# LeapLabTHU/LAUDNet

Measured on AMD Instinct MI355X. Metric: images/sec, LAUD-ResNet101 @224 bs256 (dynamic-inference hot path), higher is better.
Workload: dtype bf16x3 (fp32 tensors; each fp32 product = 3 bf16 MFMA products of hi/lo splits, fp32 accumulate)

## Files before the change

laudnet_amd/csrc/ldn_dense.hip:

```cpp
#include "ldn_common.h"
#include "ldn_dense_plan.h"
#include <type_traits>

namespace ldn {

struct DenseArgs {
    const float* a; int lda;
    const int32_t* a_rows; const int32_t* m_count; int m_cap;
    const unsigned char* ws;
    int cin, cout;
    const float* scale; const float* shift; int relu;
    const int32_t* relu_if_neg; const int32_t* out_rows;
    const float* residual; int ldr; float* out; int ldo;
    int taps;
    int shift_classes; const int32_t* pix_map;
    int Hi, Wi, Ho, Wo, stride;
    const float* post_sub;
    const float* chmask; int rows_per_img;
    int mtn, ntn;
    const float* ln_stats; const float* ln_c1;
    float* pool; int pool_gy, pool_gx, pool_Sx;
    const float* a_gate; int gate_rows;
};

__device__ __attribute__((aligned(16))) float g_dense_zero[2048] = {0.f};
#ifdef LDN_TRACE
__device__ unsigned long long* g_dense_trace = nullptr;
#define DT(x) x = __builtin_amdgcn_s_memtime();
#else
#define DT(x)
#endif

#ifndef LDN_DENSE_ABLATE
#define LDN_DENSE_ABLATE 0
#endif
__device__ __forceinline__ void dma16_abl(const void* gsrc, unsigned lds_base) {
#if LDN_DENSE_ABLATE & 1
    return;
#endif
#if LDN_DENSE_ABLATE & 2
    gsrc = g_dense_zero;
#endif
    dma16(gsrc, lds_base);
}

constexpr int D_ROWS_MAX = 256;
constexpr int D_ROW_RELU = 1 << 30;

template <int NSUB, bool T9, bool FULL, bool OF, bool FEAT = true>
__device__ __forceinline__ void dense_epilogue(const DenseArgs& p, f32x16 (&acc)[NSUB], const int* s_arow, const int* s_orow, const int* s_cls,
                                               float* scr, int wave, int lane, int n0, int nsub) {
    const int l31 = lane & 31, h = lane >> 5;
    const int trw = lane >> 3, tc = lane & 7;
    int orw[4];
#pragma unroll
    for (int it = 0; it < 4; ++it) orw[it] = s_orow[wave * 32 + trw + 8 * it];
    const bool gelu = FEAT && p.relu == 3;
    long poff = -1;
    const int pb3 = (lane >> 3) & 1, pb4 = (lane >> 4) & 1;
    if constexpr (!T9 && FULL) {
        if (p.pool) {
            const int it_sel = p.pool_gy * p.pool_gx == 16 ? (lane >= 32 ? 2 : 0) : pb3 + 2 * pb4;
            const int o = it_sel == 0 ? orw[0] : it_sel == 1 ? orw[1] : it_sel == 2 ? orw[2] : orw[3];
            if (o >= 0 && (p.pool_gy * p.pool_gx == 4 || (lane & 0x18) == 0)) {
                const int f = o & (D_ROW_RELU - 1), hw = p.Ho * p.Wo;
                const int b = f / hw, pix = f - b * hw, y = pix / p.Wo, x = pix - y * p.Wo;
                poff = ((long)b * (p.Ho / p.pool_gy) * p.pool_Sx + (y / p.pool_gy) * p.pool_Sx + x / p.pool_gx) * p.cout;
            }
        }
    }
    auto load_res = [&](int j, f32x4 (&res)[4], f32x4& sc, f32x4& sh, f32x4& ps) {
        const int cb = n0 + 32 * j + tc * 4;
        const bool cok = FULL || cb < p.cout;
#pragma unroll
        for (int it = 0; it < 4; ++it) {
            const float* src = (p.residual && orw[it] >= 0 && cok) ? p.residual + (size_t)(orw[it] & (D_ROW_RELU - 1)) * p.ldr + cb : g_dense_zero;
            res[it] = *reinterpret_cast<const f32x4*>(src);
        }
        sh = cok ? *reinterpret_cast<const f32x4*>(p.shift + cb) : f32x4{0.f, 0.f, 0.f, 0.f};
        sc = (p.scale && cok) ? *reinterpret_cast<const f32x4*>(p.scale + cb) : f32x4{1.f, 1.f, 1.f, 1.f};
        ps = (FEAT && p.post_sub && cok) ? *reinterpret_cast<const f32x4*>(p.post_sub + cb) : f32x4{0.f, 0.f, 0.f, 0.f};
    };
#pragma unroll
    for (int j = 0; j < NSUB; ++j) {
        if (j >= nsub) continue;
        f32x4 res[4], sc, sh, ps;
        load_res(j, res, sc, sh, ps);
        f32x4 cm[4];
        const bool cok = FULL || n0 + 32 * j + tc * 4 < p.cout;
        float2 lst[4];
        f32x4 lc1 = {0.f, 0.f, 0.f, 0.f};
        if (FEAT && p.ln_stats) {
#pragma unroll
            for (int it = 0; it < 4; ++it) {
                const int ar = s_arow[wave * 32 + trw + 8 * it];
                lst[it] = ar >= 0 ? *reinterpret_cast<const float2*>(p.ln_stats + 2 * (size_t)ar) : float2{0.f, 1.f};
            }
            if (cok) lc1 = *reinterpret_cast<const f32x4*>(p.ln_c1 + n0 + 32 * j + tc * 4);
        }
#pragma unroll
        for (int it = 0; it < 4; ++it) {
            const float* src = (FEAT && p.chmask && orw[it] >= 0 && cok) ? p.chmask + (size_t)((orw[it] & (D_ROW_RELU - 1)) / p.rows_per_img) * p.cout + n0 + 32 * j + tc * 4
                                                          : nullptr;
            cm[it] = src ? *reinterpret_cast<const f32x4*>(src) : f32x4{1.f, 1.f, 1.f, 1.f};
        }
#pragma unroll
        for (int q4 = 0; q4 < 4; ++q4) {
            const f32x4 v = {acc[j][4 * q4], acc[j][4 * q4 + 1], acc[j][4 * q4 + 2], acc[j][4 * q4 + 3]};
            *reinterpret_cast<f32x4*>(scr + l31 * 32 + (((2 * q4 + h) ^ (l31 & 7)) << 2)) = v;
        }
        asm volatile("s_waitcnt lgkmcnt(0)" ::: "memory");
        __builtin_amdgcn_wave_barrier();
        asm volatile("" : "+v"(res[0]), "+v"(res[1]), "+v"(res[2]), "+v"(res[3]), "+v"(sc), "+v"(sh), "+v"(ps));
        asm volatile("" : "+v"(cm[0]), "+v"(cm[1]), "+v"(cm[2]), "+v"(cm[3]));
        f32x4 xs4[4];
#pragma unroll
        for (int it = 0; it < 4; ++it) {
            const int row = trw + 8 * it;
            f32x4 x = *reinterpret_cast<const f32x4*>(scr + row * 32 + ((tc ^ (row & 7)) << 2));
            const f32x4 shr = (T9 && p.shift_classes > 1 && cok) ? *reinterpret_cast<const f32x4*>(p.shift + s_cls[wave * 32 + row] + n0 + 32 * j + tc * 4) : sh;
            if (FEAT && p.ln_stats) x = (x - lc1 * lst[it].x) * lst[it].y;
            x = x * sc + shr + res[it];
            if (orw[it] & D_ROW_RELU) {
#pragma unroll
                for (int e = 0; e < 4; ++e) x[e] = fmaxf(x[e], 0.f);
            }
            if (gelu) {
#pragma unroll
                for (int e = 0; e < 4; ++e) x[e] = 0.5f * x[e] * (1.f + erff(x[e] * 0.70710678118654752f));
            }
            x = (x - ps) * cm[it];
            if constexpr (OF) {
                const bool odd = tc & 1;
                const u32x4 o = presplit_store_quad(x, odd);
                if (orw[it] >= 0 && cok)
                    store16(reinterpret_cast<unsigned char*>(p.out) + ((size_t)(orw[it] & (D_ROW_RELU - 1)) * p.ldo + n0 + 32 * j + (tc & ~1) * 4) * 4 + (odd ? 16 : 0), o);
            } else {
                if (orw[it] >= 0 && cok)
                    store16(p.out + (size_t)(orw[it] & (D_ROW_RELU - 1)) * p.ldo + n0 + 32 * j + tc * 4, x);
            }
            xs4[it] = x;
        }
        if constexpr (!T9 && FULL) {
            if (p.pool) {
                auto swap32_sum = [](float a, float b) {
                    asm volatile("s_nop 1\n\tv_permlane32_swap_b32 %0, %1" : "+v"(a), "+v"(b));
                    return a + b;
                };
                auto swap16_sum = [](float a, float b) {
                    asm volatile("s_nop 1\n\tv_permlane16_swap_b32 %0, %1" : "+v"(a), "+v"(b));
                    return a + b;
                };
                auto ror8 = [](float a) { return __builtin_bit_cast(float, __builtin_amdgcn_update_dpp(0, __builtin_bit_cast(int, a), 0x128, 0xf, 0xf, false)); };
                f32x4 m;
                if (p.pool_gy * p.pool_gx == 16) {
                    const f32x4 sa = xs4[0] + xs4[1], sb = xs4[2] + xs4[3];
#pragma unroll
                    for (int e = 0; e < 4; ++e) {
                        float v = swap32_sum(sa[e], sb[e]);
                        v = swap16_sum(v, v);
                        m[e] = v + ror8(v);
                    }
                    m *= 0.0625f;
                } else {
                    const f32x4 k0 = pb3 ? xs4[1] : xs4[0], g0 = pb3 ? xs4[0] : xs4[1];
                    const f32x4 k2 = pb3 ? xs4[3] : xs4[2], g2 = pb3 ? xs4[2] : xs4[3];
#pragma unroll
                    for (int e = 0; e < 4; ++e) {
                        const float k01 = k0[e] + ror8(g0[e]), k23 = k2[e] + ror8(g2[e]);
                        m[e] = swap16_sum(k01, k23);
                    }
                    m *= 0.25f;
                }
                if (poff >= 0) *reinterpret_cast<f32x4*>(p.pool + poff + n0 + 32 * j + tc * 4) = m;
            }
        }
        asm volatile("s_waitcnt lgkmcnt(0)" ::: "memory");
        __builtin_amdgcn_wave_barrier();
    }
}

template <int NSUB, bool T9, bool FULL, bool F32 = false, int R = 256, bool PS = false, bool OF = false>
__global__ __launch_bounds__(2 * R, 2) void k_dense(const DenseArgs p) {
    constexpr int NT = NSUB * 32;
    constexpr int D = (NSUB >= 6 || R == 128) ? 2 : 3;
    constexpr int D_ROWS = R, NTHR = 2 * R, WR = R / 4;
    constexpr int SLOT = (D_ROWS + NT) * 128;
    constexpr int NWI = (NT + WR - 1) / WR;
    extern __shared__ __attribute__((aligned(16))) unsigned char smem[];
    int* const s_arow = reinterpret_cast<int*>(smem);
    int* const s_orow = s_arow + D_ROWS;
    int* const s_cls = s_orow + D_ROWS;
    int* const s_atap = s_cls + D_ROWS;
    unsigned char* const s_ring = smem + (T9 ? 12 : 2) * D_ROWS * 4;

    const int tid = threadIdx.x, lane = tid & 63;
    const int wave = __builtin_amdgcn_readfirstlane(tid >> 6);
    const int l31 = lane & 31, h = lane >> 5;
    const int xcd = blockIdx.x & 7, slot_i = blockIdx.x >> 3;
    const int nt = slot_i % p.ntn, mt = (slot_i / p.ntn) * 8 + xcd;
    if (mt >= p.mtn) return;
    const int M = p.m_count ? min(p.m_count[0], p.m_cap) : p.m_cap;
    const int m0 = mt * D_ROWS;
    if (m0 >= M) return;
    const int rows = min(D_ROWS, M - m0);
    const int n0 = nt * NT;
    const int nsub = FULL ? NSUB : min(NSUB, ceil_div(p.cout - n0, 32));

    if (tid < D_ROWS) {
        int ar = -1, orw = -1;
        if (tid < rows) {
            ar = (p.a_rows && !T9) ? p.a_rows[m0 + tid] : m0 + tid;
            orw = p.out_rows ? p.out_rows[m0 + tid] : m0 + tid;
            if (p.relu == 1 || (p.relu == 2 && p.relu_if_neg[m0 + tid] < 0)) orw |= D_ROW_RELU;
        }
        int cls = 0;
        if (T9 && tid < rows && p.shift_classes > 1) {
            const int q = p.pix_map[m0 + tid] % (p.Ho * p.Wo);
            const int oy = q / p.Wo, ox = q - oy * p.Wo;
            const int top = oy * p.stride - 1 < 0, bot = oy * p.stride + 1 >= p.Hi;
            const int lef = ox * p.stride - 1 < 0, rig = ox * p.stride + 1 >= p.Wi;
            cls = ((top | (bot << 1)) * 4 + (lef | (rig << 1))) * p.cout;
        }
        LDN_DCHECK(tid >= rows || (ar >= -1 && (orw & (D_ROW_RELU - 1)) >= 0), 501);
        s_arow[tid] = ar;
        s_orow[tid] = orw;
        if (T9) s_cls[tid] = cls;
    }
    if (T9) {
        constexpr int NE = (D_ROWS * 9 + NTHR - 1) / NTHR;
        int tv[NE];
#pragma unroll
        for (int u = 0; u < NE; ++u) {
            const int i = tid + NTHR * u, r = i / 9;
            tv[u] = (i < D_ROWS * 9 && r < rows) ? p.a_rows[(size_t)(m0 + r) * 9 + (i - r * 9)] : -1;
        }
#pragma unroll
        for (int u = 0; u < NE; ++u)
            if (tid + NTHR * u < D_ROWS * 9) s_atap[tid + NTHR * u] = tv[u];
    }
    __syncthreads();

    const bool active = wave * 32 < rows;
    const int cpt = ceil_div(p.cin, 32);
    const int wrow = (T9 ? 9 : 1) * (p.cin / 8);
    const int nchunks = (T9 ? 9 : 1) * cpt;
    const unsigned lds_ring = lds_off(s_ring);
    const int nwi = (NT % WR == 0 || (NWI - 1) * WR + wave * 8 < NT) ? NWI : NWI - 1;
    const int per_chunk = (active ? 4 : 0) + nwi;
    long asrc[4];
#pragma unroll
    for (int i = 0; i < 4; ++i) {
        const int ar = s_arow[wave * 32 + i * 8 + (lane >> 3)];
        asrc[i] = ar >= 0 ? (long)ar * p.lda : -1;
    }
    auto dma_chunk = [&](int c) {
        const unsigned slot = lds_ring + (c % D) * SLOT;
        const int tap = T9 ? c / cpt : 0, ck = c - tap * cpt;
        if (active) {
#pragma unroll
            for (int i = 0; i < 4; ++i) {
                const int r = wave * 32 + i * 8 + (lane >> 3);
                const int ls = (lane & 7) ^ ((r >> 1) & 7);
                long off = asrc[i];
                if (T9) {
                    const int ar = s_atap[r * 9 + tap];
// ... 92 lines not shown
        wait_vm_rt<16, 0>(per_chunk * (D - 2));
        DT(d1)
        lds_barrier();
        DT(d2)
        if (!(FULL && active)) { if (c + D - 1 < nchunks) dma_chunk(c + D - 1); else dma_dummy(c + D - 1); }
        DT(d3)
        if (!active) continue;
        const unsigned char* ws = s_ring + (c % D) * SLOT + D_ROWS * 128;
        if (!PRE) load_b(c);
#define LDN_DENSE_STEP(ACC_, AH_, AL_, BH_, BL_) \
        if constexpr (F32) { \
            const f32x4 a0_ = __builtin_bit_cast(f32x4, AH_), a1_ = __builtin_bit_cast(f32x4, AL_); \
            const f32x4 b0_ = __builtin_bit_cast(f32x4, BH_), b1_ = __builtin_bit_cast(f32x4, BL_); \
            _Pragma("unroll") for (int i_ = 0; i_ < 4; ++i_) ACC_ = __builtin_amdgcn_mfma_f32_32x32x2f32(a0_[i_], b0_[i_], ACC_, 0, 0, 0); \
            _Pragma("unroll") for (int i_ = 0; i_ < 4; ++i_) ACC_ = __builtin_amdgcn_mfma_f32_32x32x2f32(a1_[i_], b1_[i_], ACC_, 0, 0, 0); \
        } else { \
            ACC_ = __builtin_amdgcn_mfma_f32_32x32x16_bf16(AL_, BH_, ACC_, 0, 0, 0); \
            ACC_ = __builtin_amdgcn_mfma_f32_32x32x16_bf16(AH_, BL_, ACC_, 0, 0, 0); \
            ACC_ = __builtin_amdgcn_mfma_f32_32x32x16_bf16(AH_, BH_, ACC_, 0, 0, 0); \
        }
#ifdef LDN_TRACE
        asm volatile("" : "+v"(bh[0]), "+v"(bl[0]), "+v"(bh[1]), "+v"(bl[1]));
        DT(d4)
#endif
        auto frag = [&](int step, bf16x8& ah, bf16x8& al) {
            const int half = step / NSUB, j = step - half * NSUB;
            const unsigned sl = 4u * half + 2u * h;
#if LDN_DENSE_ABLATE & 8
            if (step > 1) return;
#endif
            ah = *reinterpret_cast<const bf16x8*>(ws + (32 * j + l31) * 128 + ((sl ^ wsw) << 4));
            al = *reinterpret_cast<const bf16x8*>(ws + (32 * j + l31) * 128 + (((sl + 1) ^ wsw) << 4));
        };
        if constexpr (FULL) {
            bf16x8 ah[2], al[2];
            frag(0, ah[0], al[0]);
            __builtin_amdgcn_sched_barrier(0);
#pragma unroll
            for (int st = 0; st < 2 * NSUB; ++st) {
                if (st + 1 < 2 * NSUB) frag(st + 1, ah[(st + 1) & 1], al[(st + 1) & 1]);
                __builtin_amdgcn_sched_barrier(0);
                const int half = st / NSUB, j = st - half * NSUB;
#if LDN_DENSE_ABLATE & 4
                asm volatile("" : "+v"(acc[j]) : "v"(al[st & 1]), "v"(ah[st & 1]), "v"(bh[half]), "v"(bl[half]));
#else
                LDN_DENSE_STEP(acc[j], ah[st & 1], al[st & 1], bh[half], bl[half])
#endif
                __builtin_amdgcn_sched_barrier(0);
                if (st < 4 + nwi) {
                    dma_one(c + D - 1, st);
                    __builtin_amdgcn_sched_barrier(0);
                }
            }
#pragma unroll
            for (int k = 2 * NSUB; k < 4 + NWI; ++k)
                if (k < 4 + nwi) dma_one(c + D - 1, k);
            if (PRE && c + 1 < nchunks) {
                wait_vm_rt<16, 0>(own_landed <= 16 ? own_landed : 0);
                load_b(c + 1);
            }
        } else {
#pragma unroll
            for (int half = 0; half < 2; ++half) {
#pragma unroll
                for (int j = 0; j < NSUB; ++j) {
                    if (j < nsub) {
                        bf16x8 ah, al;
                        frag(half * NSUB + j, ah, al);
                        LDN_DENSE_STEP(acc[j], ah, al, bh[half], bl[half])
                    }
                }
            }
        }
#ifdef LDN_TRACE
        asm volatile("" : "+v"(acc[0]));
        DT(d5)
        a_wait += d1 - d0; a_bar += d2 - d1; a_issue += d3 - d2; a_prep += d4 - d3; a_mfma += d5 - d4;
#endif
    }
#undef LDN_DENSE_STEP
#ifdef LDN_TRACE
    DT(d_loop)
#endif
    wait_vm<0>();
    lds_barrier();
    if (!active) return;

    dense_epilogue<NSUB, T9, FULL, OF>(p, acc, s_arow, s_orow, s_cls, reinterpret_cast<float*>(s_ring + wave * 4096), wave, lane, n0, nsub);
#if defined(LDN_TRACE)
    if (g_dense_trace && lane == 0) {
        unsigned long long dend;
        DT(dend)
        unsigned long long* r = g_dense_trace + ((size_t)blockIdx.x * 8 + wave) * 8;
        r[0] = a_wait; r[1] = a_bar; r[2] = a_issue; r[3] = a_prep; r[4] = a_mfma; r[5] = d_loop - d_start; r[6] = dend - d_loop; r[7] = nchunks;
    }
#endif
}

template <int NSUB, bool T9, bool PS, bool OF, bool FEAT = false, bool RAG = false, bool AG = false>
__global__ __launch_bounds__(512, 2) void k_dense2(const DenseArgs p) {
    static_assert(!RAG || (!T9 && !PS && !OF), "the ragged form is the plain 1x1");
    static_assert(!AG || (!T9 && !PS), "the gated form reads fp32 rows of a 1x1");
    constexpr int NT = NSUB * 32;
    constexpr int KS = NSUB <= 4 ? 64 : 32;
    constexpr int SPS = KS / 32;
    constexpr int WROWB = KS * 4;
    constexpr int UPR = WROWB / 16;
    constexpr int RPI = 1024 / WROWB;
    constexpr int NWI = (NT + 8 * RPI - 1) / (8 * RPI);
    constexpr int WSLOT = NWI * 8 * 1024;
    constexpr int RSLOT = 32 * 128;
    constexpr int D_ROWS = 256, NST = 2 * NSUB;
    extern __shared__ __attribute__((aligned(16))) unsigned char smem[];
    int* const s_arow = reinterpret_cast<int*>(smem);
    int* const s_orow = s_arow + D_ROWS;
    int* const s_cls = s_orow + D_ROWS;
    int* const s_atap = s_cls + D_ROWS;
    unsigned char* const s_w = smem + (T9 ? 12 : 2) * D_ROWS * 4;
    unsigned char* const s_r = s_w + 2 * WSLOT;
    float* const s_gate = reinterpret_cast<float*>(s_r + 8 * 2 * RSLOT);

    const int tid = threadIdx.x, lane = tid & 63;
    const int wave = __builtin_amdgcn_readfirstlane(tid >> 6);
    const int l31 = lane & 31, h = lane >> 5;
    const int xcd = blockIdx.x & 7, slot_i = blockIdx.x >> 3;
    const int nt = slot_i % p.ntn, mt = (slot_i / p.ntn) * 8 + xcd;
    if (mt >= p.mtn) return;
    const int M = p.m_count ? min(p.m_count[0], p.m_cap) : p.m_cap;
    const int m0 = mt * D_ROWS;
    if (m0 >= M) return;
    const int rows = min(D_ROWS, M - m0);
    const int n0 = nt * NT;

    if (tid < D_ROWS) {
        int ar = -1, orw = -1;
        if (tid < rows) {
            ar = (p.a_rows && !T9) ? p.a_rows[m0 + tid] : m0 + tid;
            orw = p.out_rows ? p.out_rows[m0 + tid] : m0 + tid;
            if (p.relu == 1 || (p.relu == 2 && p.relu_if_neg[m0 + tid] < 0)) orw |= D_ROW_RELU;
        }
        int cls = 0;
        if (T9 && tid < rows && p.shift_classes > 1) {
            const int q = p.pix_map[m0 + tid] % (p.Ho * p.Wo);
            const int oy = q / p.Wo, ox = q - oy * p.Wo;
            const int top = oy * p.stride - 1 < 0, bot = oy * p.stride + 1 >= p.Hi;
            const int lef = ox * p.stride - 1 < 0, rig = ox * p.stride + 1 >= p.Wi;
            cls = ((top | (bot << 1)) * 4 + (lef | (rig << 1))) * p.cout;
        }
        LDN_DCHECK(tid >= rows || (ar >= -1 && (orw & (D_ROW_RELU - 1)) >= 0), 501);
        s_arow[tid] = ar;
        s_orow[tid] = orw;
        if (T9) s_cls[tid] = cls;
    }
    if (T9) {
        constexpr int NE = (D_ROWS * 9 + 511) / 512;
        int tv[NE];
#pragma unroll
        for (int u = 0; u < NE; ++u) {
            const int i = tid + 512 * u, r = i / 9;
            tv[u] = (i < D_ROWS * 9 && r < rows) ? p.a_rows[(size_t)(m0 + r) * 9 + (i - r * 9)] : -1;
        }
#pragma unroll
        for (int u = 0; u < NE; ++u)
            if (tid + 512 * u < D_ROWS * 9) s_atap[tid + 512 * u] = tv[u];
    }
    int goff = 0;
    if constexpr (AG) {
        const int gld = round_up(p.cin, 32), q4 = gld >> 2;
        const int slot0 = m0 / p.gate_rows, nsl = (m0 + rows - 1) / p.gate_rows - slot0 + 1;
        for (int i = tid; i < nsl * q4; i += 512) {
            const int sl = i / q4, k = (i - sl * q4) * 4;
            reinterpret_cast<f32x4*>(s_gate)[i] = k < p.cin ? *reinterpret_cast<const f32x4*>(p.a_gate + (size_t)(slot0 + sl) * p.cin + k) : f32x4{0.f, 0.f, 0.f, 0.f};
        }
        goff = ((m0 + min(wave * 32 + (lane & 31), rows - 1)) / p.gate_rows - slot0) * gld + 8 * (lane >> 5);
    }
    __syncthreads();

    const bool active = wave * 32 < rows;
    const int cpt = RAG ? ceil_div(p.cin, 32) : p.cin >> 5;
    const int nsubc = (T9 ? 9 : 1) * cpt, nstep = RAG ? ceil_div(nsubc, SPS) : nsubc / SPS;
    const int nsub_t = RAG ? min(NSUB, ceil_div(p.cout - n0, 32)) : NSUB;
    const long wrow = (long)(T9 ? 9 : 1) * p.cin * 4;
    const unsigned lds_w = lds_off(s_w), lds_r = lds_off(s_r) + (unsigned)wave * 2u * RSLOT;
// ... 108 lines not shown

    load_tap(0);
#pragma unroll
    for (int k = 0; k < NWI; ++k) dma_w(0, k);
#pragma unroll
    for (int k = 0; k < 4; ++k) dma_r(0, k);
    next_r();
#pragma unroll
    for (int k = 0; k < 4; ++k) dma_r(1, k);
    next_r();
    wait_vm<4>();
    read_b(0, bh[0], bl[0]);
    split_b(0, bh[0], bl[0]);
    split_b(1, bh[0], bl[0]);
    asm volatile("s_waitcnt lgkmcnt(0)" ::: "memory");
    __builtin_amdgcn_sched_barrier(0);
#pragma unroll
    for (int k = 0; k < 4; ++k) dma_r(2, k);
    next_r();
    if constexpr (SPS == 1) wait_vm<4>();

    auto step = [&](int S, auto cur0_c) {
        constexpr int CUR0 = decltype(cur0_c)::value;
        wait_vm<SPS == 2 ? 8 : 4>();
        lds_barrier();
        const unsigned char* wsl = s_w + (S & 1) * WSLOT + l31 * WROWB;
        auto body = [&](auto sub_c, auto cur_c) {
            constexpr int sub = decltype(sub_c)::value, CUR = decltype(cur_c)::value;
            const int s = SPS * S + sub;
            auto frag = [&](int st, bf16x8& ah, bf16x8& al) {
                const int half = st / NSUB, j = st - half * NSUB;
                const unsigned uu = 2u * ((SPS == 2 ? 4u * sub : 0u) + 2u * half + h);
                ah = *reinterpret_cast<const bf16x8*>(wsl + j * (32 * WROWB) + ((uu ^ wsw) << 4));
                al = *reinterpret_cast<const bf16x8*>(wsl + j * (32 * WROWB) + (((uu + 1) ^ wsw) << 4));
            };
            bf16x8 ah[2], al[2];
            frag(0, ah[0], al[0]);
            __builtin_amdgcn_sched_barrier(0);
            constexpr int rd_at = sub == 0 ? (NWI < NST - 1 ? NWI : NST - 2) : 0;
            int r_done = 0, w_done = 0, sp_done = PS ? 2 : 0;
#pragma unroll
            for (int st = 0; st < NST; ++st) {
                if (st + 1 < NST) frag(st + 1, ah[(st + 1) & 1], al[(st + 1) & 1]);
                __builtin_amdgcn_sched_barrier(0);
                const int half = st / NSUB, j = st - half * NSUB;
                if (!RAG || j < nsub_t) {
                    acc[j] = __builtin_amdgcn_mfma_f32_32x32x16_bf16(al[st & 1], bh[CUR][half], acc[j], 0, 0, 0);
                    acc[j] = __builtin_amdgcn_mfma_f32_32x32x16_bf16(ah[st & 1], bl[CUR][half], acc[j], 0, 0, 0);
                    acc[j] = __builtin_amdgcn_mfma_f32_32x32x16_bf16(ah[st & 1], bh[CUR][half], acc[j], 0, 0, 0);
                }
                __builtin_amdgcn_sched_barrier(0);
                if (sub == 0 && st < rd_at) {
                    if (w_done < NWI) dma_w(S + 1, w_done++);
                } else if (st == rd_at) {
                    if (sub == 0)
                        while (w_done < NWI) dma_w(S + 1, w_done++);
                    wait_vm<SPS == 2 ? 4 + NWI : 4 + 2 * NWI>();
                    read_b(s + 1, bh[CUR ^ 1], bl[CUR ^ 1]);
                } else if (sp_done < 2) {
                    split_b(sp_done++, bh[CUR ^ 1], bl[CUR ^ 1]);
                } else {
                    if (r_done == 0) asm volatile("s_waitcnt lgkmcnt(0)" ::: "memory");
                    if (r_done < 4) dma_r(s + 3, r_done++);
                }
                __builtin_amdgcn_sched_barrier(0);
            }
            while (sp_done < 2) split_b(sp_done++, bh[CUR ^ 1], bl[CUR ^ 1]);
            if (r_done == 0) asm volatile("s_waitcnt lgkmcnt(0)" ::: "memory");
            while (r_done < 4) dma_r(s + 3, r_done++);
            next_r();
            __builtin_amdgcn_sched_barrier(0);
        };
        body(std::integral_constant<int, 0>{}, std::integral_constant<int, CUR0>{});
        if constexpr (SPS == 2) body(std::integral_constant<int, 1>{}, std::integral_constant<int, CUR0 ^ 1>{});
    };
    if constexpr (SPS == 2) {
        for (int S = 0; S < nstep; ++S) step(S, std::integral_constant<int, 0>{});
    } else {
        for (int S = 0; S < nstep; S += 2) {
            step(S, std::integral_constant<int, 0>{});
            if (!RAG || S + 1 < nstep) step(S + 1, std::integral_constant<int, 1>{});
        }
    }
    wait_vm<0>();
    asm volatile("s_waitcnt lgkmcnt(0)" ::: "memory");
    dense_epilogue<NSUB, T9, !RAG, OF, FEAT || T9>(p, acc, s_arow, s_orow, s_cls, reinterpret_cast<float*>(my_r), wave, lane, n0, nsub_t);
}

__global__ __launch_bounds__(256) void k_row_stats(const float* __restrict__ x, int ld, int rows, int C, float eps, float* __restrict__ stats,
                                                    const int32_t* __restrict__ list, const int32_t* __restrict__ count) {
    const int lane = threadIdx.x & 63;
    int r = blockIdx.x * 4 + (threadIdx.x >> 6);
    if (list) {
        if (r >= min(*count, rows)) return;
        r = list[r];
    }
    if (r >= rows) return;
    const float* xr = x + (size_t)r * ld;
    f32x4 v[8];
    float s = 0.f;
#pragma unroll
    for (int i = 0; i < 8; ++i) {
        const int c = (i * 64 + lane) * 4;
        v[i] = c < C ? *reinterpret_cast<const f32x4*>(xr + c) : f32x4{0.f, 0.f, 0.f, 0.f};
        s += (v[i][0] + v[i][1]) + (v[i][2] + v[i][3]);
    }
#pragma unroll
    for (int o = 32; o > 0; o >>= 1) s += __shfl_xor(s, o, 64);
    const float mean = s / (float)C;
    float q = 0.f;
#pragma unroll
    for (int i = 0; i < 8; ++i) {
        const int c = (i * 64 + lane) * 4;
        if (c < C) {
#pragma unroll
            for (int e = 0; e < 4; ++e) { const float d = v[i][e] - mean; q += d * d; }
        }
    }
#pragma unroll
    for (int o = 32; o > 0; o >>= 1) q += __shfl_xor(q, o, 64);
    if (lane == 0) *reinterpret_cast<float2*>(stats + 2 * (size_t)r) = float2{mean, rsqrtf(q / (float)C + eps)};
}

LDN_DEFINE_TU_VIOLATIONS(tu_violations_dense)

static int launch_rows(void (*kernel)(const DenseArgs), const char* name, int r, int nt, unsigned threads, size_t lds, DenseArgs& a, hipStream_t st) {
    a.ntn = ceil_div(a.cout, nt);
    a.mtn = ceil_div(a.m_cap, r);
    LDN_REQUIRE(allow_dynamic_lds(reinterpret_cast<const void*>(kernel), lds), "%s: cannot reserve %zu B of LDS", name, lds);
    hipLaunchKernelGGL(kernel, dim3((unsigned)round_up(a.mtn, 8) * a.ntn), dim3(threads), lds, st, a);
    LDN_CHECK_LAUNCH(name);
    return LDN_OK;
}

template <int NSUB, bool T9, bool FULL, bool F32, int R, bool PS, bool OF>
static int launch_dense_f(DenseArgs& a, hipStream_t st) {
    constexpr int NT = NSUB * 32, D = (NSUB >= 6 || R == 128) ? 2 : 3;
    return launch_rows(&k_dense<NSUB, T9, FULL, F32, R, PS, OF>, "k_dense", R, NT, 2 * R, (size_t)(T9 ? 12 : 2) * R * 4 + (size_t)D * (R + NT) * 128, a, st);
}

template <int NSUB, bool T9, bool PS, bool OF, bool FEAT, bool RAG, bool AG>
static int launch_dense2(DenseArgs& a, hipStream_t st) {
    constexpr int NT = NSUB * 32, KS = NSUB <= 4 ? 64 : 32, WROWB = KS * 4, RPI = 1024 / WROWB, NWI = (NT + 8 * RPI - 1) / (8 * RPI);
    const size_t lds = (size_t)(T9 ? 12 : 2) * 256 * 4 + 2 * (size_t)NWI * 8 * 1024 + 8 * 2 * (size_t)32 * 128 +
                       (AG ? (size_t)dense_gate_bytes(a.gate_rows, a.cin) : 0);
    return launch_rows(&k_dense2<NSUB, T9, PS, OF, FEAT, RAG, AG>, "k_dense2", 256, NT, 512, lds, a, st);
}

static int launch_dense_plan(const DensePlan& plan, DenseArgs& a, hipStream_t st) {
#define LDN_D1(...) if (plan == LDN_DENSE_ROW1(__VA_ARGS__)) return launch_dense_f<__VA_ARGS__>(a, st);
#define LDN_D2(...) if (plan == LDN_DENSE_ROW2(__VA_ARGS__)) return launch_dense2<__VA_ARGS__>(a, st);
    LDN_DENSE_KERNELS(LDN_D1, LDN_D2)
#undef LDN_D1
#undef LDN_D2
    LDN_REQUIRE(false, "ldn_conv_rows: %s is not built (taps %d, cin %d, cout %d, m_cap %d)", dense_plan_name(plan).c_str(), a.taps, a.cin, a.cout, a.m_cap);
}

}

using namespace ldn;

#ifdef LDN_TRACE
extern "C" int ldn_debug_set_dense_trace(void* buf) {
    unsigned long long* q = static_cast<unsigned long long*>(buf);
    return hipMemcpyToSymbol(HIP_SYMBOL(g_dense_trace), &q, sizeof(q)) == hipSuccess ? 0 : -2;
}
#endif

// ... 160 lines not shown
```

laudnet_amd/csrc/ldn_rows3.hip:

```cpp
#include "ldn_common.h"

namespace ldn {

struct Rows3Args {
    const unsigned char* a; long lda;
    const int32_t* nbr;
    const int32_t* m_count; int m_cap;
    const unsigned char* ws;
    int cin, cout;
    const float* scale; const float* shift; int relu;
    unsigned char* out; long ldo;
    int mtn, ntn;
};

constexpr int ROWS3_MAX_CIN = 2048;
__device__ __attribute__((aligned(16))) float g_rows3_zero[ROWS3_MAX_CIN] = {0.f};
#ifdef LDN_TRACE
__device__ unsigned long long* g_rows3_trace = nullptr;
#define RT(x) x = __builtin_amdgcn_s_memtime();
#else
#define RT(x)
#endif

__device__ __forceinline__ void dma16_m0(const void* gsrc, unsigned lds_base) {
// ... 117 lines not shown

#ifdef R3_PRIO
    if (wave >= 4) __builtin_amdgcn_s_setprio(1);
#endif
    load_tap(0);
#pragma unroll
    for (int k = 0; k < NWI; ++k) dma_w(0, k);
#pragma unroll
    for (int k = 0; k < 4; ++k) dma_r(0, k);
    next_r();
#pragma unroll
    for (int k = 0; k < 4; ++k) dma_r(1, k);
    next_r();
    wait_vm<4>();
    load_b(0, bh[0], bl[0]);
    wait_lgkm0();
    __builtin_amdgcn_sched_barrier(0);
#pragma unroll
    for (int k = 0; k < 4; ++k) dma_r(2, k);
    next_r();

#ifdef LDN_TRACE
    unsigned long long t0, t1, t2, t3, a_wait = 0, a_bar = 0, a_body = 0, t_start, t_loop;
    RT(t_start)
#endif
    for (int S = 0; S < nsup; ++S) {
        RT(t0)
        wait_vm<8>();
        RT(t1)
        lds_barrier();
        RT(t2)
        const unsigned char* wsl = s_w + (S & 1) * WSLOT + l31 * 256;
#pragma unroll
        for (int sub = 0; sub < 2; ++sub) {
            const int s = 2 * S + sub;
            auto frag = [&](int st, bf16x8& ah, bf16x8& al) {
                const int half = st / NSUB, j = st - half * NSUB;
                const unsigned uu = 2u * (4u * sub + 2u * half + h);
                ah = *reinterpret_cast<const bf16x8*>(wsl + j * (32 * 256) + ((uu ^ wsw) << 4));
                al = *reinterpret_cast<const bf16x8*>(wsl + j * (32 * 256) + (((uu + 1) ^ wsw) << 4));
            };
            bf16x8 ah[2], al[2];
            frag(0, ah[0], al[0]);
            __builtin_amdgcn_sched_barrier(0);
            constexpr int NST = 2 * NSUB;
            const int rd_at = sub == 0 ? (NWI < NST - 1 ? NWI : NST - 2) : 0;
            int r_done = 0, w_done = 0;
#pragma unroll
            for (int st = 0; st < NST; ++st) {
                if (st + 1 < NST) frag(st + 1, ah[(st + 1) & 1], al[(st + 1) & 1]);
                __builtin_amdgcn_sched_barrier(0);
                const int half = st / NSUB, j = st - half * NSUB;
                acc[j] = __builtin_amdgcn_mfma_f32_32x32x16_bf16(al[st & 1], bh[sub][half], acc[j], 0, 0, 0);
                acc[j] = __builtin_amdgcn_mfma_f32_32x32x16_bf16(ah[st & 1], bl[sub][half], acc[j], 0, 0, 0);
                acc[j] = __builtin_amdgcn_mfma_f32_32x32x16_bf16(ah[st & 1], bh[sub][half], acc[j], 0, 0, 0);
                __builtin_amdgcn_sched_barrier(0);
                if (sub == 0 && st < rd_at) {
                    if (w_done < NWI) dma_w(S + 1, w_done++);
                } else if (st == rd_at) {
                    if (sub == 0)
                        while (w_done < NWI) dma_w(S + 1, w_done++);
                    wait_vm<4 + NWI>();
                    load_b(s + 1, bh[sub ^ 1], bl[sub ^ 1]);
                } else {
                    if (r_done == 0) wait_lgkm0();
                    if (r_done < 4) dma_r(s + 3, r_done++);
                }
                __builtin_amdgcn_sched_barrier(0);
            }
            if (r_done == 0) wait_lgkm0();
            while (r_done < 4) dma_r(s + 3, r_done++);
            next_r();
            __builtin_amdgcn_sched_barrier(0);
        }
#ifdef LDN_TRACE
        asm volatile("" : "+v"(acc[0]));
        RT(t3)
        a_wait += t1 - t0; a_bar += t2 - t1; a_body += t3 - t2;
#endif
    }
#ifdef LDN_TRACE
    RT(t_loop)
#endif
    wait_vm<0>();
    wait_lgkm0();

    float* const scr = reinterpret_cast<float*>(my_r);
    const int trw = lane >> 3, tc = lane & 7;
#pragma unroll
    for (int j = 0; j < NSUB; ++j) {
        const int cb = n0 + 32 * j + tc * 4;
        const f32x4 sh = *reinterpret_cast<const f32x4*>(p.shift + cb);
        const f32x4 sc = p.scale ? *reinterpret_cast<const f32x4*>(p.scale + cb) : f32x4{1.f, 1.f, 1.f, 1.f};
#pragma unroll
        for (int q4 = 0; q4 < 4; ++q4) {
            const f32x4 v = {acc[j][4 * q4], acc[j][4 * q4 + 1], acc[j][4 * q4 + 2], acc[j][4 * q4 + 3]};
            *reinterpret_cast<f32x4*>(scr + l31 * 32 + (((2 * q4 + h) ^ (l31 & 7)) << 2)) = v;
        }
        wait_lgkm0();
        __builtin_amdgcn_wave_barrier();
#pragma unroll
        for (int it = 0; it < 4; ++it) {
            const int row = trw + 8 * it;
            f32x4 x = *reinterpret_cast<const f32x4*>(scr + row * 32 + ((tc ^ (row & 7)) << 2));
            x = x * sc + sh;
            if (p.relu) {
#pragma unroll
                for (int e = 0; e < 4; ++e) x[e] = fmaxf(x[e], 0.f);
            }
            const bool ok = wave * 32 + row < rows;
            unsigned char* orow = p.out + (size_t)(m0 + wave * 32 + row) * p.ldo;
            if constexpr (OF) {
                const bool odd = tc & 1;
                const u32x4 o = presplit_store_quad(x, odd);
                if (ok) store16(orow + (size_t)(n0 + 32 * j + (tc & ~1) * 4) * 4 + (odd ? 16 : 0), o);
            } else {
                if (ok) store16(orow + (size_t)cb * 4, x);
            }
        }
        wait_lgkm0();
        __builtin_amdgcn_wave_barrier();
    }
#ifdef LDN_TRACE
    if (g_rows3_trace && lane == 0) {
        unsigned long long t_end;
        RT(t_end)
        unsigned long long* r = g_rows3_trace + ((size_t)blockIdx.x * 8 + wave) * 8;
        r[0] = a_wait; r[1] = a_bar; r[2] = a_body; r[3] = 0; r[4] = 0; r[5] = t_loop - t_start; r[6] = t_end - t_loop; r[7] = nsup;
    }
#endif
}

LDN_DEFINE_TU_VIOLATIONS(tu_violations_rows3)

template <int NSUB, bool OF>
static int launch_rows3(Rows3Args& a, hipStream_t st) {
    constexpr int NT = NSUB * 32;
    const size_t lds = (size_t)R3_ROWS * 9 * 4 + 2 * (size_t)NT * 256 + 8 * 2 * (size_t)32 * 128;
    a.ntn = a.cout / NT;
    a.mtn = ceil_div(a.m_cap, R3_ROWS);
    LDN_REQUIRE(allow_dynamic_lds(reinterpret_cast<const void*>(&k_rows3<NSUB, OF>), lds), "k_rows3: cannot reserve %zu B of LDS", lds);
    const unsigned grid = (unsigned)round_up(a.mtn, 8) * a.ntn;
    hipLaunchKernelGGL((k_rows3<NSUB, OF>), dim3(grid), dim3(512), lds, st, a);
    LDN_CHECK_LAUNCH("k_rows3");
    return LDN_OK;
}

}

using namespace ldn;

#ifdef LDN_TRACE
extern "C" int ldn_debug_set_rows3_trace(void* buf) {
    unsigned long long* q = static_cast<unsigned long long*>(buf);
    return hipMemcpyToSymbol(HIP_SYMBOL(g_rows3_trace), &q, sizeof(q)) == hipSuccess ? 0 : -2;
}
#endif

extern "C" int ldn_conv3x3_rows_ps(const void* a_presplit, int lda, const int32_t* nbr, const int32_t* m_count, int m_cap, const void* w_split,
                                   int cin, int cout, const float* scale, const float* shift, int relu, void* out, int ldo, int out_presplit,
                                   int rows_hint, void* stream) {
    LDN_REQUIRE(a_presplit && nbr && w_split && shift && out, "ldn_conv3x3_rows_ps: null pointer");
    LDN_REQUIRE(cin > 0 && cin % 64 == 0 && cout > 0 && cout % 64 == 0, "ldn_conv3x3_rows_ps: cin and cout must be multiples of 64 (got %d, %d)", cin, cout);
    LDN_REQUIRE(cin <= ldn::ROWS3_MAX_CIN, "ldn_conv3x3_rows_ps: cin must be <= %d (a missing neighbour is sourced from a zero row of that width; got %d -- use ldn_conv_rows_split(taps = 9))", ldn::ROWS3_MAX_CIN, cin);
    LDN_REQUIRE(lda >= cin && lda % 4 == 0 && ldo >= cout && ldo % 4 == 0, "ldn_conv3x3_rows_ps: strides (in 4-byte elements) must be multiples of 4 and cover the row");
    LDN_REQUIRE((uintptr_t)a_presplit % 16 == 0 && (uintptr_t)w_split % 16 == 0 && (uintptr_t)out % 16 == 0 && (uintptr_t)shift % 16 == 0 &&
                (uintptr_t)scale % 16 == 0, "ldn_conv3x3_rows_ps: pointers must be 16-byte aligned");
    LDN_REQUIRE(relu == 0 || relu == 1, "ldn_conv3x3_rows_ps: relu must be 0 or 1");
    if (m_cap <= 0) return LDN_OK;
    Rows3Args d{static_cast<const unsigned char*>(a_presplit), (long)lda * 4, nbr, m_count, m_cap, static_cast<const unsigned char*>(w_split), cin, cout,
                scale, shift, relu, static_cast<unsigned char*>(out), (long)ldo * 4, 0, 0};
    hipStream_t st = static_cast<hipStream_t>(stream);
    const long rows = !m_count ? (long)m_cap : (rows_hint >= 0 ? (rows_hint < m_cap ? rows_hint : m_cap) : -1);
    bool narrow = cout % 128 != 0;
    if (!narrow && rows > 0) {
        const long wg128 = ((rows + R3_ROWS - 1) / R3_ROWS) * (cout / 128);
// ... 6 lines not shown
```

Measured before the change: 23120.

## Batch epilogue loads ahead of a single wait and stage per-column params in LDS

The dense epilogue now DMAs the per-column scale, shift, post_sub and ln_c1 vectors into LDS once. It also issues residual, channel-mask and class-shift loads for several sub-tiles ahead of a single wait, so each sub-tile no longer pays its own global load latency. The batch size comes from a register-budget heuristic, and launch bounds now vary occupancy with NSUB. The rows3 epilogue likewise hoists its shift and scale loads before the final wait. This adds register pressure and template complexity, plus a larger per-wave LDS scratch in k_dense that relies on the ring being big enough.

```diff
diff --git a/laudnet_amd/csrc/ldn_dense.hip b/laudnet_amd/csrc/ldn_dense.hip
--- a/laudnet_amd/csrc/ldn_dense.hip
+++ b/laudnet_amd/csrc/ldn_dense.hip
@@ -47,9 +47,32 @@
 constexpr int D_ROWS_MAX = 256;
 constexpr int D_ROW_RELU = 1 << 30;
 
-template <int NSUB, bool T9, bool FULL, bool OF, bool FEAT = true>
+__device__ __attribute__((aligned(16))) float g_dense_one[4] = {1.f, 1.f, 1.f, 1.f};
+template <int NSUB, bool FULL, bool FEAT>
+__device__ __forceinline__ void dense_cols_dma(const DenseArgs& p, int lane, int n0, unsigned lds_col) {
+    const int cb = n0 + 4 * lane;
+    const bool ok = lane < NSUB * 8 && (FULL || cb < p.cout);
+    dma16((ok && p.scale) ? p.scale + cb : g_dense_one, lds_col);
+    dma16(ok ? p.shift + cb : g_dense_zero, lds_col + 1024u);
+    if constexpr (FEAT) {
+        dma16((ok && p.post_sub) ? p.post_sub + cb : g_dense_zero, lds_col + 2048u);
+        dma16((ok && p.ln_stats) ? p.ln_c1 + cb : g_dense_zero, lds_col + 3072u);
+    }
+}
+
+constexpr int dense_epi_batch(int nsub, int nk, bool feat, int done) {
+    if (nk == 0) return nsub - done;
+    const int ceiling = nsub <= 2 ? 128 : nsub <= 5 ? 168 : 256;
+    const int blocks = (ceiling - (feat ? 90 : 60)) / 16 - (nsub - done);
+    const int b = blocks / nk;
+    return b < 1 ? 1 : b > nsub - done ? nsub - done : b;
+}
+
+template <int NSUB, bool T9, bool FULL, bool OF, bool FEAT = true, bool SYNC = false>
 __device__ __forceinline__ void dense_epilogue(const DenseArgs& p, f32x16 (&acc)[NSUB], const int* s_arow, const int* s_orow, const int* s_cls,
                                                float* scr, int wave, int lane, int n0, int nsub) {
+    float* const col = scr + 1024;
+    const unsigned lds_col = (unsigned)__builtin_amdgcn_readfirstlane((int)lds_off(col));
     const int l31 = lane & 31, h = lane >> 5;
     const int trw = lane >> 3, tc = lane & 7;
     int orw[4];
@@ -69,40 +92,85 @@
             }
         }
     }
-    auto load_res = [&](int j, f32x4 (&res)[4], f32x4& sc, f32x4& sh, f32x4& ps) {
-        const int cb = n0 + 32 * j + tc * 4;
-        const bool cok = FULL || cb < p.cout;
+    if constexpr (!SYNC) dense_cols_dma<NSUB, FULL, FEAT>(p, lane, n0, lds_col);
+    const bool has_ln = FEAT && p.ln_stats;
+    float2 lst[4];
+    if (has_ln) {
 #pragma unroll
         for (int it = 0; it < 4; ++it) {
-            const float* src = (p.residual && orw[it] >= 0 && cok) ? p.residual + (size_t)(orw[it] & (D_ROW_RELU - 1)) * p.ldr + cb : g_dense_zero;
-            res[it] = *reinterpret_cast<const f32x4*>(src);
-        }
-        sh = cok ? *reinterpret_cast<const f32x4*>(p.shift + cb) : f32x4{0.f, 0.f, 0.f, 0.f};
-        sc = (p.scale && cok) ? *reinterpret_cast<const f32x4*>(p.scale + cb) : f32x4{1.f, 1.f, 1.f, 1.f};
-        ps = (FEAT && p.post_sub && cok) ? *reinterpret_cast<const f32x4*>(p.post_sub + cb) : f32x4{0.f, 0.f, 0.f, 0.f};
-    };
-#pragma unroll
-    for (int j = 0; j < NSUB; ++j) {
-        if (j >= nsub) continue;
-        f32x4 res[4], sc, sh, ps;
-        load_res(j, res, sc, sh, ps);
-        f32x4 cm[4];
+            const int ar = s_arow[wave * 32 + trw + 8 * it];
+            lst[it] = ar >= 0 ? *reinterpret_cast<const float2*>(p.ln_stats + 2 * (size_t)ar) : float2{0.f, 1.f};
+        }
+    }
+    auto settle = [&]() __attribute__((always_inline)) {
+        wait_vm<0>();
+        if constexpr (SYNC) {
+            lds_barrier();
+            dense_cols_dma<NSUB, FULL, FEAT>(p, lane, n0, lds_col);
+            wait_vm<0>();
+        }
+        if (has_ln) asm volatile("" : "+v"(lst[0]), "+v"(lst[1]), "+v"(lst[2]), "+v"(lst[3]));
+        wait_lgkm0();
+        __builtin_amdgcn_wave_barrier();
+    };
+    const bool has_res = p.residual != nullptr, has_cm = FEAT && p.chmask, has_cls = T9 && p.shift_classes > 1;
+    auto run = [&](auto res_c, auto cm_c, auto cls_c) __attribute__((always_inline)) {
+    constexpr bool RES = decltype(res_c)::value, CM = decltype(cm_c)::value, CLS = decltype(cls_c)::value;
+    constexpr bool CLS_LATE = CLS && SYNC && NSUB == 2;
+    constexpr int NK = RES + CM + (CLS && !CLS_LATE);
+    const bool hres = NK == 1 ? RES : has_res, hcm = NK == 1 ? CM : has_cm, hcls = (NK == 1 && !CLS_LATE) ? CLS : has_cls;
+    f32x4 res[RES ? NSUB : 1][4], cm[CM ? NSUB : 1][4], cs[CLS ? NSUB : 1][4];
+    auto batch = [&](auto self, auto j0_c) __attribute__((always_inline)) -> void {
+    constexpr int j0 = decltype(j0_c)::value;
+    if constexpr (j0 < NSUB) {
+    constexpr int B = dense_epi_batch(NSUB, NK, FEAT, j0);
+    if constexpr (NK > 0) {
+#pragma unroll
+        for (int b = 0; b < B; ++b) {
+            const int j = j0 + b;
+            if (j >= NSUB || j >= nsub) continue;
+            const int cb = n0 + 32 * j + tc * 4;
+            const bool cok = FULL || cb < p.cout;
+#pragma unroll
+            for (int it = 0; it < 4; ++it) {
+                const bool ok = orw[it] >= 0 && cok;
+                const size_t orow = (size_t)(orw[it] & (D_ROW_RELU - 1));
+                if constexpr (RES) {
+                    res[j][it] = f32x4{0.f, 0.f, 0.f, 0.f};
+                    if (hres) res[j][it] = *reinterpret_cast<const f32x4*>(ok ? p.residual + orow * p.ldr + cb : g_dense_zero);
+                }
+                if constexpr (CM) {
+                    cm[j][it] = f32x4{1.f, 1.f, 1.f, 1.f};
+                    if (hcm && ok) cm[j][it] = *reinterpret_cast<const f32x4*>(p.chmask + (orow / p.rows_per_img) * p.cout + cb);
+                }
+                if constexpr (CLS && !CLS_LATE) {
+                    cs[j][it] = f32x4{0.f, 0.f, 0.f, 0.f};
+                    if (hcls && cok) cs[j][it] = *reinterpret_cast<const f32x4*>(p.shift + s_cls[wave * 32 + trw + 8 * it] + cb);
+                }
+            }
+        }
+    }
+    if (j0 == 0) settle();
+    if constexpr (NK > 0) {
+#pragma unroll
+        for (int b = 0; b < B; ++b) {
+            const int j = j0 + b;
+            if (j >= NSUB || j >= nsub) continue;
+            if constexpr (RES) asm volatile("" : "+v"(res[j][0]), "+v"(res[j][1]), "+v"(res[j][2]), "+v"(res[j][3]));
+            if constexpr (CM) asm volatile("" : "+v"(cm[j][0]), "+v"(cm[j][1]), "+v"(cm[j][2]), "+v"(cm[j][3]));
+            if constexpr (CLS && !CLS_LATE) asm volatile("" : "+v"(cs[j][0]), "+v"(cs[j][1]), "+v"(cs[j][2]), "+v"(cs[j][3]));
+        }
+    }
+#pragma unroll
+    for (int b = 0; b < B; ++b) {
+        const int j = j0 + b;
+        if (j >= NSUB || j >= nsub) continue;
         const bool cok = FULL || n0 + 32 * j + tc * 4 < p.cout;
-        float2 lst[4];
-        f32x4 lc1 = {0.f, 0.f, 0.f, 0.f};
-        if (FEAT && p.ln_stats) {
-#pragma unroll
-            for (int it = 0; it < 4; ++it) {
-                const int ar = s_arow[wave * 32 + trw + 8 * it];
-                lst[it] = ar >= 0 ? *reinterpret_cast<const float2*>(p.ln_stats + 2 * (size_t)ar) : float2{0.f, 1.f};
-            }
-            if (cok) lc1 = *reinterpret_cast<const f32x4*>(p.ln_c1 + n0 + 32 * j + tc * 4);
-        }
-#pragma unroll
-        for (int it = 0; it < 4; ++it) {
-            const float* src = (FEAT && p.chmask && orw[it] >= 0 && cok) ? p.chmask + (size_t)((orw[it] & (D_ROW_RELU - 1)) / p.rows_per_img) * p.cout + n0 + 32 * j + tc * 4
-                                                          : nullptr;
-            cm[it] = src ? *reinterpret_cast<const f32x4*>(src) : f32x4{1.f, 1.f, 1.f, 1.f};
+        const f32x4 sc = *reinterpret_cast<const f32x4*>(col + 32 * j + tc * 4), sh = *reinterpret_cast<const f32x4*>(col + 256 + 32 * j + tc * 4);
+        f32x4 ps = {0.f, 0.f, 0.f, 0.f}, lc1 = {0.f, 0.f, 0.f, 0.f};
+        if constexpr (FEAT) {
+            ps = *reinterpret_cast<const f32x4*>(col + 512 + 32 * j + tc * 4);
+            lc1 = *reinterpret_cast<const f32x4*>(col + 768 + 32 * j + tc * 4);
         }
 #pragma unroll
         for (int q4 = 0; q4 < 4; ++q4) {
@@ -111,16 +179,22 @@
         }
         asm volatile("s_waitcnt lgkmcnt(0)" ::: "memory");
         __builtin_amdgcn_wave_barrier();
-        asm volatile("" : "+v"(res[0]), "+v"(res[1]), "+v"(res[2]), "+v"(res[3]), "+v"(sc), "+v"(sh), "+v"(ps));
-        asm volatile("" : "+v"(cm[0]), "+v"(cm[1]), "+v"(cm[2]), "+v"(cm[3]));
         f32x4 xs4[4];
 #pragma unroll
         for (int it = 0; it < 4; ++it) {
             const int row = trw + 8 * it;
             f32x4 x = *reinterpret_cast<const f32x4*>(scr + row * 32 + ((tc ^ (row & 7)) << 2));
-            const f32x4 shr = (T9 && p.shift_classes > 1 && cok) ? *reinterpret_cast<const f32x4*>(p.shift + s_cls[wave * 32 + row] + n0 + 32 * j + tc * 4) : sh;
-            if (FEAT && p.ln_stats) x = (x - lc1 * lst[it].x) * lst[it].y;
-            x = x * sc + shr + res[it];
+            f32x4 shr = sh, rs = {0.f, 0.f, 0.f, 0.f}, cmv = {1.f, 1.f, 1.f, 1.f};
+            if constexpr (CLS) {
+                if (hcls && cok) {
+                    if constexpr (CLS_LATE) shr = *reinterpret_cast<const f32x4*>(p.shift + s_cls[wave * 32 + row] + n0 + 32 * j + tc * 4);
+                    else shr = cs[j][it];
+                }
+            }
+            if constexpr (RES) rs = res[j][it];
+            if constexpr (CM) cmv = cm[j][it];
+            if (has_ln) x = (x - lc1 * lst[it].x) * lst[it].y;
+            x = x * sc + shr + rs;
             if (orw[it] & D_ROW_RELU) {
 #pragma unroll
                 for (int e = 0; e < 4; ++e) x[e] = fmaxf(x[e], 0.f);
@@ -129,7 +203,7 @@
 #pragma unroll
                 for (int e = 0; e < 4; ++e) x[e] = 0.5f * x[e] * (1.f + erff(x[e] * 0.70710678118654752f));
             }
-            x = (x - ps) * cm[it];
+            x = (x - ps) * cmv;
             if constexpr (OF) {
                 const bool odd = tc & 1;
                 const u32x4 o = presplit_store_quad(x, odd);
@@ -178,10 +252,19 @@
         asm volatile("s_waitcnt lgkmcnt(0)" ::: "memory");
         __builtin_amdgcn_wave_barrier();
     }
-}
+    self(self, std::integral_constant<int, j0 + B>{});
+    }
+    };
+    batch(batch, std::integral_constant<int, 0>{});
+    };
+    if (!has_res && !has_cm && !has_cls) run(std::false_type{}, std::false_type{}, std::false_type{});
+    else run(std::true_type{}, std::bool_constant<FEAT>{}, std::bool_constant<T9>{});
+}
+
+constexpr int dense_min_waves(int nsub, bool low) { return nsub <= 2 ? (low ? 3 : 4) : nsub <= 5 ? (low ? 2 : 3) : 2; }
 
 template <int NSUB, bool T9, bool FULL, bool F32 = false, int R = 256, bool PS = false, bool OF = false>
-__global__ __launch_bounds__(2 * R, 2) void k_dense(const DenseArgs p) {
+__global__ __launch_bounds__(2 * R, dense_min_waves(NSUB, NSUB == 5 && FULL)) void k_dense(const DenseArgs p) {
     constexpr int NT = NSUB * 32;
     constexpr int D = (NSUB >= 6 || R == 128) ? 2 : 3;
     constexpr int D_ROWS = R, NTHR = 2 * R, WR = R / 4;
@@ -440,11 +523,14 @@
 #ifdef LDN_TRACE
     DT(d_loop)
 #endif
-    wait_vm<0>();
-    lds_barrier();
-    if (!active) return;
-
-    dense_epilogue<NSUB, T9, FULL, OF>(p, acc, s_arow, s_orow, s_cls, reinterpret_cast<float*>(s_ring + wave * 4096), wave, lane, n0, nsub);
+    if (!active) {
+        wait_vm<0>();
+        lds_barrier();
+        return;
+    }
+
+    static_assert(D * SLOT >= (NTHR / 64) * 8192, "the ring holds every wave's epilogue scratch");
+    dense_epilogue<NSUB, T9, FULL, OF, true, true>(p, acc, s_arow, s_orow, s_cls, reinterpret_cast<float*>(s_ring + wave * 8192), wave, lane, n0, nsub);
 #if defined(LDN_TRACE)
     if (g_dense_trace && lane == 0) {
         unsigned long long dend;
@@ -456,7 +542,7 @@
 }
 
 template <int NSUB, bool T9, bool PS, bool OF, bool FEAT = false, bool RAG = false, bool AG = false>
-__global__ __launch_bounds__(512, 2) void k_dense2(const DenseArgs p) {
+__global__ __launch_bounds__(512, dense_min_waves(NSUB, AG || (T9 && NSUB == 2))) void k_dense2(const DenseArgs p) {
     static_assert(!RAG || (!T9 && !PS && !OF), "the ragged form is the plain 1x1");
     static_assert(!AG || (!T9 && !PS), "the gated form reads fp32 rows of a 1x1");
     constexpr int NT = NSUB * 32;
@@ -731,8 +817,6 @@
             if (!RAG || S + 1 < nstep) step(S + 1, std::integral_constant<int, 1>{});
         }
     }
-    wait_vm<0>();
-    asm volatile("s_waitcnt lgkmcnt(0)" ::: "memory");
     dense_epilogue<NSUB, T9, !RAG, OF, FEAT || T9>(p, acc, s_arow, s_orow, s_cls, reinterpret_cast<float*>(my_r), wave, lane, n0, nsub_t);
 }
 
diff --git a/laudnet_amd/csrc/ldn_rows3.hip b/laudnet_amd/csrc/ldn_rows3.hip
--- a/laudnet_amd/csrc/ldn_rows3.hip
+++ b/laudnet_amd/csrc/ldn_rows3.hip
@@ -223,16 +223,23 @@
 #ifdef LDN_TRACE
     RT(t_loop)
 #endif
+    float* const scr = reinterpret_cast<float*>(my_r);
+    const int trw = lane >> 3, tc = lane & 7;
+    f32x4 sh_t[NSUB], sc_t[NSUB];
+#pragma unroll
+    for (int j = 0; j < NSUB; ++j) {
+        const int cb = n0 + 32 * j + tc * 4;
+        sh_t[j] = *reinterpret_cast<const f32x4*>(p.shift + cb);
+        sc_t[j] = p.scale ? *reinterpret_cast<const f32x4*>(p.scale + cb) : f32x4{1.f, 1.f, 1.f, 1.f};
+    }
     wait_vm<0>();
     wait_lgkm0();
-
-    float* const scr = reinterpret_cast<float*>(my_r);
-    const int trw = lane >> 3, tc = lane & 7;
+#pragma unroll
+    for (int j = 0; j < NSUB; ++j) asm volatile("" : "+v"(sh_t[j]), "+v"(sc_t[j]));
 #pragma unroll
     for (int j = 0; j < NSUB; ++j) {
         const int cb = n0 + 32 * j + tc * 4;
-        const f32x4 sh = *reinterpret_cast<const f32x4*>(p.shift + cb);
-        const f32x4 sc = p.scale ? *reinterpret_cast<const f32x4*>(p.scale + cb) : f32x4{1.f, 1.f, 1.f, 1.f};
+        const f32x4 sh = sh_t[j], sc = sc_t[j];
 #pragma unroll
         for (int q4 = 0; q4 < 4; ++q4) {
             const f32x4 v = {acc[j][4 * q4], acc[j][4 * q4 + 1], acc[j][4 * q4 + 2], acc[j][4 * q4 + 3]};
```

Result: no change. 23320 (median of 2 runs) (+0.8%).
